# pedrocr/imagepipe

Hardware: AMD Instinct MI355X
Metric: megapixels/sec full raw->sRGB pipe, 100 MP f32 frame (higher is better)
Workload: dtype f32

## Files before the change

bindings/rust/imagepipe_amd_sys.rs:

```rust
#![allow(non_camel_case_types, dead_code)]
use std::os::raw::{c_char, c_int, c_uint, c_void};

pub const IPK_OK: c_int = 0;
pub const IPK_NOOP: c_int = 1;
pub const IPK_ERR_NOT_INIT: c_int = -1;
pub const IPK_ERR_INVALID: c_int = -2;
pub const IPK_ERR_HIP: c_int = -3;
pub const IPK_ERR_NO_DEVICE: c_int = -4;
pub const IPK_ERR_UNSUPPORTED: c_int = -5;
pub const IPK_ERR_NOMEM: c_int = -6;

pub const IPK_OR_NORMAL: c_int = 0;
pub const IPK_OR_HFLIP: c_int = 1;
pub const IPK_OR_ROT180: c_int = 2;
pub const IPK_OR_VFLIP: c_int = 3;
pub const IPK_OR_TRANSPOSE: c_int = 4;
pub const IPK_OR_ROT90: c_int = 5;
pub const IPK_OR_TRANSVERSE: c_int = 6;
pub const IPK_OR_ROT270: c_int = 7;
pub const IPK_OR_UNKNOWN: c_int = 8;

pub const IPK_ROT_NORMAL: c_int = 0;
pub const IPK_ROT_90: c_int = 1;
pub const IPK_ROT_180: c_int = 2;
// ... 230 lines not shown
  pub fn ipk_host_output16bit(src: *const f32, n: usize, dst: *mut u16) -> c_int;
  pub fn ipk_host_raw_to_srgb(p: *const IpkFusedParams, src: *const c_void, dst: *mut c_void) -> c_int;
  pub fn ipk_selftest_cdiv(c: f32, variant: c_int, lo: f32, hi: f32, include_special: c_int, n_bad: *mut u64, first_bad_bits: *mut u32) -> c_int;
  pub fn ipk_selftest_lut_weight(n_bad: *mut u64, first_bad_bits: *mut u32) -> c_int;
  pub fn ipk_selftest_clamp01(n_bad: *mut u64, first_bad_bits: *mut u32) -> c_int;
  pub fn ipk_copy_probe(src: *const c_void, dst: *mut c_void, bytes: usize, stream: *mut c_void) -> c_int;
  pub fn ipk_mix_probe(src: *const c_void, dst: *mut c_void, src_bytes: usize, stream: *mut c_void) -> c_int;
  pub fn ipk_clock_probe(out2_dev: *mut u64, spin_us: u32, stream: *mut c_void) -> c_int;
  pub fn ipk_stream_probe(p: *const IpkFusedParams, src: *const c_void, dst: *mut c_void, stream: *mut c_void) -> c_int;
  pub fn ipk_selftest_spline3(exposure: f32, points: *const f32, npoints: c_int, n_bad: *mut u64, first_bad_bits: *mut u32) -> c_int;
  pub fn ipk_selftest_quant8(variant: c_int, n_bad: *mut u64, first_bad_bits: *mut u32) -> c_int;
  pub fn ipk_selftest_q8(n_bad: *mut u64, first_bad_bits: *mut u32) -> c_int;
  pub fn ipk_selftest_quant16(n_bad: *mut u64, first_bad_bits: *mut u32) -> c_int;
  pub fn ipk_selftest_cbrtf(r#in: *const f32, out: *mut f32, n: usize, variant: c_int, stream: *mut c_void) -> c_int;
  pub fn ipk_selftest_task_queue(enabled: c_int) -> c_int;
  pub fn ipk_selftest_cache_put(cache: *mut IpkCache, key32: *const u8, bytes: usize) -> c_int;
  pub fn ipk_selftest_sha256(data: *const c_void, n: usize, out32: *mut u8) -> c_int;
}
```

imagepipe_amd/_lib.py:

```python
import ctypes as C
import os

_HERE = os.path.dirname(os.path.abspath(__file__))
SO_PATH = os.environ.get("IPK_SO_OVERRIDE") or os.path.join(_HERE, "libimagepipe_amd.so")

IPK_OK, IPK_NOOP = 0, 1
SRC_U16, SRC_F32, SRC_RGB8, SRC_RGB16 = 0, 1, 2, 3
OUT_F32, OUT_U8, OUT_U16 = 0, 1, 2
SCHED_AUTO, SCHED_SPLIT = 0, 1
OR_NORMAL, OR_HFLIP, OR_ROT180, OR_VFLIP, OR_TRANSPOSE, OR_ROT90, OR_TRANSVERSE, OR_ROT270, OR_UNKNOWN = range(9)
ROT_NORMAL, ROT_90, ROT_180, ROT_270 = range(4)

_sz = C.c_size_t
_vp = C.c_void_p
_fp = C.POINTER(C.c_float)
_szp = C.POINTER(C.c_size_t)
_i64 = C.c_int64


class _SizedDesc(C.Structure):

    def __init__(self, *a, **k):
        super().__init__(*a, **k)
        self.struct_size = C.sizeof(self)
# ... 141 lines not shown
    "ipk_host_raw_to_srgb": (C.c_int, [C.POINTER(FusedParams), _vp, _vp]),
    "ipk_selftest_cdiv": (C.c_int, [C.c_float, C.c_int, C.c_float, C.c_float, C.c_int, C.POINTER(C.c_uint64), C.POINTER(C.c_uint32)]),
    "ipk_selftest_lut_weight": (C.c_int, [C.POINTER(C.c_uint64), C.POINTER(C.c_uint32)]),
    "ipk_selftest_clamp01": (C.c_int, [C.POINTER(C.c_uint64), C.POINTER(C.c_uint32)]),
    "ipk_abi_sizeof": (_sz, [C.c_int]),
    "ipk_copy_probe": (C.c_int, [_vp, _vp, _sz, _vp]),
    "ipk_mix_probe": (C.c_int, [_vp, _vp, _sz, _vp]),
    "ipk_clock_probe": (C.c_int, [_vp, C.c_uint32, _vp]),
    "ipk_stream_probe": (C.c_int, [C.POINTER(FusedParams), _vp, _vp, _vp]),
    "ipk_selftest_spline3": (C.c_int, [C.c_float, _fp, C.c_int, C.POINTER(C.c_uint64), C.POINTER(C.c_uint32)]),
    "ipk_selftest_quant8": (C.c_int, [C.c_int, C.POINTER(C.c_uint64), C.POINTER(C.c_uint32)]),
    "ipk_selftest_q8": (C.c_int, [C.POINTER(C.c_uint64), C.POINTER(C.c_uint32)]),
    "ipk_selftest_quant16": (C.c_int, [C.POINTER(C.c_uint64), C.POINTER(C.c_uint32)]),
    "ipk_selftest_cbrtf": (C.c_int, [_vp, _vp, _sz, C.c_int, _vp]),
    "ipk_selftest_task_queue": (C.c_int, [C.c_int]),
    "ipk_selftest_cache_put": (C.c_int, [_vp, C.c_char_p, _sz]),
    "ipk_selftest_sha256": (C.c_int, [C.c_char_p, _sz, C.c_char_p]),
    "ipk_pointwise_chain": (C.c_int, [_vp, _sz, _sz, C.c_int, _fp, _fp, C.c_float, _fp, C.c_int, C.c_int, _vp, _vp]),
    "ipk_pointwise_chain_out": (C.c_int, [_vp, _sz, _sz, C.c_int, _fp, _fp, C.c_float, _fp, C.c_int, C.c_int, C.c_int, _vp, _vp]),
    "ipk_raster_to_srgb": (C.c_int, [_vp, C.c_int, _sz, _sz, _fp, _fp, C.c_float, _fp, C.c_int, C.c_int, C.c_int, _vp, _vp]),
    "ipk_pipeline_takes_fastpath": (C.c_int, [C.POINTER(PipelineDesc), C.c_int]),
    "ipk_pipeline_fuses_rotatecrop": (C.c_int, [C.POINTER(PipelineDesc), C.c_int]),
    "ipk_pipeline_hashes": (C.c_int, [C.POINTER(PipelineDesc), C.c_int, C.c_uint64, C.c_char_p]),
    "ipk_cache_new": (C.c_int, [_sz, C.POINTER(C.c_void_p)]),
    "ipk_cache_free": (C.c_int, [_vp]),
    "ipk_cache_clear": (C.c_int, [_vp]),
    "ipk_cache_contains": (C.c_int, [_vp, C.c_char_p]),
    "ipk_cache_stats": (C.c_int, [_vp, C.POINTER(_sz), C.POINTER(_sz), C.POINTER(C.c_uint64), C.POINTER(C.c_uint64), C.POINTER(C.c_uint64)]),
    "ipk_cache_get": (C.c_int, [_vp, C.c_char_p, C.POINTER(C.c_void_p), C.POINTER(_sz), C.POINTER(_sz), C.POINTER(_sz), C.POINTER(C.c_int)]),
    "ipk_timing_begin": (C.c_int, []),
# ... 52 lines not shown
```

imagepipe_amd/csrc/ipk_api.cpp:

```cpp
#include <hip/hip_runtime_api.h>

#include <algorithm>
#include <cmath>
#include <cstdarg>
#include <cstdio>
#include <cstddef>
#include <cstring>
#include <atomic>
#include <map>
#include <memory>
#include <mutex>
#include <string>
#include <thread>
#include <vector>

#include "../../include/imagepipe_amd.h"
#include "ipk_hash.hpp"
#include "ipk_host.hpp"
#include "ipk_internal.hpp"
#include "ipk_launch.hpp"

namespace {

thread_local char g_err[512] = "";
// ... 1181 lines not shown
  REQUIRE_INIT();
  if (!src || !dst || (bytes & 15) || ((uintptr_t)src & 15) || ((uintptr_t)dst & 15)) return fail(IPK_ERR_INVALID, "ipk_copy_probe wants 16-byte aligned buffers and a multiple of 16 bytes");
  ipk::launch_copy_probe(src, dst, bytes, cx().num_cus, S(stream)); HIPCHK(hipGetLastError());
  return IPK_OK;
}
int ipk_mix_probe(const void *src, void *dst, size_t src_bytes, void *stream) {
  REQUIRE_INIT();
  if (!src || !dst || (src_bytes & 4095) || ((uintptr_t)src & 15) || ((uintptr_t)dst & 15)) return fail(IPK_ERR_INVALID, "ipk_mix_probe wants 16-byte aligned buffers and a multiple of 4096 source bytes (whole blocks)");
  ipk::launch_mix_probe(src, dst, src_bytes, S(stream)); HIPCHK(hipGetLastError());
  return IPK_OK;
}
int ipk_clock_probe(uint64_t *out2_dev, uint32_t spin_us, void *stream) {
  REQUIRE_INIT();
  if (!out2_dev || spin_us == 0 || spin_us > 2000000u) return fail(IPK_ERR_INVALID, "ipk_clock_probe: null output or a spin outside (0, 2 s]");
  ipk::launch_clock_probe(out2_dev, (unsigned long long)spin_us * 100ull, S(stream)); HIPCHK(hipGetLastError());
  return IPK_OK;
}
int ipk_selftest_task_queue(int enabled) { REQUIRE_INIT(); ipk::selftest_task_queue(enabled != 0); return IPK_OK; }
int ipk_selftest_spline3(float exposure, const float *points, int npoints, uint64_t *n_bad, uint32_t *first_bad_bits) {
  REQUIRE_INIT();
  if (!n_bad || (npoints > 0 && !points)) return fail(IPK_ERR_INVALID, "bad selftest arguments");
  ipk::Spline sp; int rc = build_curve(exposure, points, npoints, sp); if (rc) return rc;
  void *dev; rc = selftest_alloc(&dev); if (rc) return rc;
  if (ipk::launch_selftest_spline3(sp, dev, nullptr) != 0) { (void)hipFree(dev); return fail(IPK_ERR_UNSUPPORTED, "the kernels keep the select form for this curve"); }
  HIPCHK(hipGetLastError());
  return selftest_collect(dev, n_bad, first_bad_bits);
}
int ipk_selftest_quant16(uint64_t *n_bad, uint32_t *first_bad_bits) {
  REQUIRE_INIT();
  if (!n_bad) return fail(IPK_ERR_INVALID, "bad selftest arguments");
// ... 1074 lines not shown
```

imagepipe_amd/csrc/ipk_kernels.hip:

```cpp
#include <hip/hip_runtime.h>
#include <stdint.h>
#include <cstring>
#include <cmath>
#include <type_traits>
#include <atomic>
#include <mutex>
#include <utility>
#include <vector>
#include "ipk_device.hpp"
#include "ipk_launch.hpp"

using namespace ipkd;

#define IPK_RARE(x) __builtin_expect(!!(x), 0)
constexpr uint32_t kSpread = 4;
constexpr uint32_t kMinTaskRows = 4;
#ifndef IPK_SPLIT_MIN_ROWS
#define IPK_SPLIT_MIN_ROWS 16u
#endif
constexpr uint32_t kStealMin = 4;

namespace ipk {

typedef LutPair LabTab;
// ... 1203 lines not shown
  uint64_t owidth;
  uint32_t row_off;
  uint32_t out_r0, out_r1;
  uint32_t n_frames;
  uint32_t *task_ctr;
  float min0, range0;
  float inv_range0;
  int exact_norm;
  int fast_ok;
  int xoff, yoff;
  ToLabParams tolab;
  Mat9 rgbm;
  int has_curve, linear;
  uint32_t n_strips, n_segs;
  uint32_t lc_base, lc_rem;
  const float *lab_table;
  const float *gam_table;
  const LutPair *lab_pairs, *gam_pairs;
  const Q8Entry *gam_q8;
  const float *gen_cells;
  uint32_t gen_pw, gen_ph;
  int gen_check;
  int px_guard;
  int ori;
  int roles[4];
  SplineDev spline;
};

struct RowWin { float l, v0, v1, v2, v3, r; };

// ... 572 lines not shown
  __shared__ __attribute__((aligned(16))) uint32_t s_stage[FULL ? 16 * STG : 4];
  if (threadIdx.x < 4) s_par[threadIdx.x] = a.tolab.mul[threadIdx.x];
  else if (threadIdx.x < 16) s_par[threadIdx.x] = a.tolab.cm[threadIdx.x - 4];
  else if (threadIdx.x < 25) s_par[threadIdx.x] = a.rgbm.m[threadIdx.x - 16];
  if (threadIdx.x < kSplineMaxKnots) fill_knots(s_knots, a.spline, (int)threadIdx.x);
  constexpr bool HAS_GRID = CM != 1 && !DEMO && !SKEL;
  __shared__ __attribute__((aligned(16))) float s_grid[HAS_GRID ? kGridFloats : 4];
  if (HAS_GRID && (CM == 2 || a.spline.grid_ok)) fill_grid(s_grid, a.spline, (int)threadIdx.x);
  __shared__ unsigned long long s_tdesc[16];
  __shared__ uint32_t s_tcur[16];
  if ((threadIdx.x & 63u) == 0) { s_tdesc[threadIdx.x >> 6] = 0ull; s_tcur[threadIdx.x >> 6] = 0u; }
  bool arrived = false;
  auto arrive = [&]() { if (!arrived) { sync_after_lds_direct(); arrived = true; } };

  const uint32_t lane = threadIdx.x & 63u;
  const uint32_t per_frame = a.n_strips * a.n_segs;
  const uint32_t n_waves = gridDim.x * (blockDim.x >> 6);
  const uint32_t n_tasks = BATCH ? per_frame * a.n_frames : per_frame;
  auto draw = [&]() -> uint32_t {
    uint32_t t = 0xFFFFFFFFu;
    if ((threadIdx.x & 63u) == 0) {
      t = n_waves + atomicAdd(a.task_ctr, 1u);
    }
    t = (uint32_t)__builtin_amdgcn_readfirstlane((int)t);
    return t;
  };
  const bool queued = a.task_ctr != nullptr && n_tasks > n_waves;
  const uint32_t wslot = threadIdx.x >> 6, nwb = blockDim.x >> 6;
  const bool steal_on = a.n_strips <= 0xFFFFu && (!BATCH || a.n_frames <= 64u);
  uint32_t tserial = 0;
  auto take_over = [&](uint32_t &frame, uint32_t &strip, uint32_t &r0, uint32_t &r1) -> bool {
    for (int attempt = 0; attempt < 4; ++attempt) {
      unsigned long long d = 0ull; uint32_t c = 0u;
// ... 12 lines not shown
      uint32_t ok = 0u;
      if (lane == 0) ok = atomicCAS(&s_tdesc[bl], dv, nv) == dv ? 1u : 0u;
      if (__builtin_amdgcn_readfirstlane((int)ok) != 0) { strip = dhi & 0xFFFFu; frame = (dhi >> 16) & 63u; r0 = mid; r1 = dlo; return true; }
    }
    return false;
  };
  const uint32_t gt0 = queued ? blockIdx.x * (blockDim.x >> 6) + (threadIdx.x >> 6)
                              : (((threadIdx.x >> 6) / kSpread) * gridDim.x + blockIdx.x) * kSpread + ((threadIdx.x >> 6) % kSpread);
  auto next_task = [&](uint32_t gt) -> uint32_t {
    if (gt >= n_tasks) return 0xFFFFFFFFu;
    if (queued) return draw();
    return (n_tasks - gt > n_waves) ? gt + n_waves : 0xFFFFFFFFu;
  };
  for (uint32_t gt = (uint32_t)__builtin_amdgcn_readfirstlane((int)gt0);; gt = next_task(gt)) {
    uint32_t frame = 0u, strip, r0, r1;
    if (gt < n_tasks) {
      frame = BATCH ? (uint32_t)__builtin_amdgcn_readfirstlane((int)(gt / per_frame)) : 0u;
      const uint32_t task = (uint32_t)__builtin_amdgcn_readfirstlane((int)(BATCH ? gt - frame * per_frame : gt));
      strip = task % a.n_strips;
      const uint32_t seg = task / a.n_strips;
      const uint32_t nrows = a.out_r1 - a.out_r0;
      r0 = a.out_r0 + (uint32_t)(((uint64_t)seg * nrows) / a.n_segs);
      r1 = a.out_r0 + (uint32_t)(((uint64_t)(seg + 1) * nrows) / a.n_segs);
    } else {
      arrive();
      if (!steal_on) break;
      if (lane == 0) __hip_atomic_store(&s_tdesc[wslot], (unsigned long long)(++tserial & 0x3FFu) << 54, __ATOMIC_RELAXED, __HIP_MEMORY_SCOPE_WORKGROUP);
      if (__builtin_amdgcn_readfirstlane(take_over(frame, strip, r0, r1) ? 1 : 0) == 0) break;
    }
    strip = (uint32_t)__builtin_amdgcn_readfirstlane((int)strip); r0 = (uint32_t)__builtin_amdgcn_readfirstlane((int)r0); r1 = (uint32_t)__builtin_amdgcn_readfirstlane((int)r1);
    if (BATCH) frame = (uint32_t)__builtin_amdgcn_readfirstlane((int)frame);
    const void *const frame_src = BATCH ? bp->src[frame] : a.src;
    void *const frame_dst = BATCH ? bp->dst[frame] : a.dst;

    const uint32_t lc0 = FULL ? 0u : strip * a.lc_base + min(strip, a.lc_rem);
    const uint32_t nl = FULL ? 64u : a.lc_base + (strip < a.lc_rem ? 1u : 0u);
    const bool lane_on = FULL ? true : lane < nl;
    const uint32_t pc0 = (WIN ? win->x0 : 0u) + (FULL ? min(strip * 256u, (WIN ? win->x1 - win->x0 : a.W) - 256u) : 4u * lc0);
    const bool win_inner = WIN && FULL && pc0 >= win->c0 && pc0 + 256u <= win->c1;
    const uint32_t col0 = pc0 + 4u * min(lane, nl - 1);
    const uint32_t nvalid = FULL ? 4u : min(4u, a.W - col0);
    const uint32_t xo = ((uint32_t)a.xoff + pc0) & 1u;
    uint32_t cxo[4] = {0, 0, 0, 0};
    if (GEN) {
      #pragma unroll
      for (int j = 0; j < 4; ++j) cxo[j] = ((col0 + j) % a.gen_pw) * kGenCellFloats;
    }
    const bool gen_guard = GEN && (sizeof(SrcT) == 4 || DEMO || a.gen_check != 0);
    if (r0 >= r1) { arrive(); continue; }
    if (steal_on && lane == 0) {
      __hip_atomic_store(&s_tdesc[wslot], (unsigned long long)(++tserial & 0x3FFu) << 54, __ATOMIC_RELAXED, __HIP_MEMORY_SCOPE_WORKGROUP);
      __hip_atomic_store(&s_tcur[wslot], r0, __ATOMIC_RELAXED, __HIP_MEMORY_SCOPE_WORKGROUP);
      __hip_atomic_store(&s_tdesc[wslot], ((unsigned long long)(((++tserial & 0x3FFu) << 22) | (frame << 16) | strip) << 32) | r1, __ATOMIC_RELEASE, __HIP_MEMORY_SCOPE_WORKGROUP);
    }

    const bool is_first = lane == 0, is_last = lane + 1 == nl;
    const bool single = FULL ? false : nl == 1;
    const int64_t hcol_want = is_first ? (int64_t)pc0 - 1 : (int64_t)pc0 + 4 * (int64_t)nl;
    const uint32_t hcol = ((is_first || is_last) && hcol_want >= 0 && hcol_want < (int64_t)a.W) ? (uint32_t)hcol_want : col0;
    const uint32_t h2col = (single && pc0 + 4u * nl < a.W) ? pc0 + 4u * nl : col0;

    const SrcT *src = reinterpret_cast<const SrcT *>(frame_src);
    const float min0 = a.min0, range0 = a.range0, inv_range0 = a.inv_range0;
    const bool exact_norm = CMN ? false : a.exact_norm != 0;
    const bool fast_ok = CMN ? true : a.fast_ok != 0, has_curve = CMN ? true : a.has_curve != 0, linear = CMN ? (OUTS == 2) : a.linear != 0;

    struct RawRowT { float v0, v1, v2, v3, h, h2; };
    auto issue_row = [&](uint32_t row) -> RawRowT {
      const SrcT *rp = src + (uint64_t)(row - a.row_off) * a.owidth;
      RawRowT t;
      load_raw4<SrcT, VEC>(rp + col0, nvalid, t.v0, t.v1, t.v2, t.v3);
// ... 41 lines not shown
      } else {
        w.v0 = rs_min(d0 / range0, 1.0f); w.v1 = rs_min(d1 / range0, 1.0f); w.v2 = rs_min(d2 / range0, 1.0f); w.v3 = rs_min(d3 / range0, 1.0f);
        h = rs_min(dh / range0, 1.0f);
        if (single) h2 = rs_min(dh2 / range0, 1.0f);
      }
      if (gen_guard) {
        flag = __builtin_amdgcn_ballot_w64(gen_sample_bad(w.v0) | gen_sample_bad(w.v1) | gen_sample_bad(w.v2) | gen_sample_bad(w.v3) |
                                           gen_sample_bad(h) | gen_sample_bad(h2)) != 0;
        if (flag && !redo) {
          w.v0 = rs_min(d0 / range0, 1.0f); w.v1 = rs_min(d1 / range0, 1.0f); w.v2 = rs_min(d2 / range0, 1.0f); w.v3 = rs_min(d3 / range0, 1.0f);
          h = rs_min(dh / range0, 1.0f);
          if (single) h2 = rs_min(dh2 / range0, 1.0f);
        }
      }
      w.l = dpp_wave_shr1(h, w.v3);
      const float rr = dpp_wave_shl1(h, w.v0);
      w.r = is_last ? (single ? h2 : h) : rr;
      return w;
    };

    const bool store_aligned = (OUTS == 0 || OUTS == 3) ? true : ((OUTS == 1) ? ((a.W & 3u) == 0) : ((a.W & 1u) == 0));
    const uint32_t Hm1 = a.H - 1, Wm1 = a.W - 1;
    const bool col_edge = lane_on && (col0 == 0 || col0 + 3 >= Wm1);

    RowWin P = {0, 0, 0, 0, 0, 0}, C, N = {0, 0, 0, 0, 0, 0};
    bool fP = false, fC = false, fN = false;
    RawRowT raw_next;
    {
      const RawRowT rp = issue_row(r0 > 0 ? r0 - 1 : 0u), rc = issue_row(r0), rn = issue_row(min(r0 + 1, Hm1));
      raw_next = issue_row(min(r0 + 2, Hm1));
      P = finish_row(rp, fP); C = finish_row(rc, fC); N = finish_row(rn, fN);
    }
    arrive();
    uint32_t ry = GEN ? r0 % a.gen_ph : 0u;
    auto compute_px = [&](const RowWin &P, const RowWin &C, const RowWin &N, const bool fP, const bool fC, const bool fN, const uint32_t r, float4 px[4]) {
      const int pr = (int)((r + (uint32_t)a.yoff) & 1u);
      const float pw[6] = {P.l, P.v0, P.v1, P.v2, P.v3, P.r};
      const float cw[6] = {C.l, C.v0, C.v1, C.v2, C.v3, C.r};
      const float nw[6] = {N.l, N.v0, N.v1, N.v2, N.v3, N.r};
      const float *rowcells = s_cells + ry * a.gen_pw * kGenCellFloats;
      if (GEN) {
        const bool literal = fP | fC | fN;
        #pragma unroll
        for (int j = 0; j < 4; ++j) {
          float t[9] = {pw[j], pw[j + 1], pw[j + 2], cw[j], cw[j + 1], cw[j + 2], nw[j], nw[j + 1], nw[j + 2]};
// ... 16 lines not shown
          px[3] = demosaic_inner_px<0, ZA>(pw[3], pw[4], pw[5], cw[3], cw[4], cw[5], nw[3], nw[4], nw[5]);
        }
      } else {
        if (xo == 0) {
          px[0] = demosaic_inner_px<2, ZA>(pw[0], pw[1], pw[2], cw[0], cw[1], cw[2], nw[0], nw[1], nw[2]);
          px[1] = demosaic_inner_px<3, ZA>(pw[1], pw[2], pw[3], cw[1], cw[2], cw[3], nw[1], nw[2], nw[3]);
          px[2] = demosaic_inner_px<2, ZA>(pw[2], pw[3], pw[4], cw[2], cw[3], cw[4], nw[2], nw[3], nw[4]);
          px[3] = demosaic_inner_px<3, ZA>(pw[3], pw[4], pw[5], cw[3], cw[4], cw[5], nw[3], nw[4], nw[5]);
        } else {
          px[0] = demosaic_inner_px<3, ZA>(pw[0], pw[1], pw[2], cw[0], cw[1], cw[2], nw[0], nw[1], nw[2]);
          px[1] = demosaic_inner_px<2, ZA>(pw[1], pw[2], pw[3], cw[1], cw[2], cw[3], nw[1], nw[2], nw[3]);
          px[2] = demosaic_inner_px<3, ZA>(pw[2], pw[3], pw[4], cw[2], cw[3], cw[4], nw[2], nw[3], nw[4]);
          px[3] = demosaic_inner_px<2, ZA>(pw[3], pw[4], pw[5], cw[3], cw[4], cw[5], nw[3], nw[4], nw[5]);
        }
      }
      const bool edge_lane = (r == 0) || (r == Hm1) || col_edge;
      if (IPK_RARE(__builtin_amdgcn_ballot_w64(edge_lane) != 0)) {
        if (edge_lane) {
          #pragma unroll
          for (int j = 0; j < 4; ++j) {
            const uint32_t c = col0 + j;
            if (c < a.W && (r == 0 || r == Hm1 || c == 0 || c == Wm1)) {
              const float t[9] = {pw[j], pw[j + 1], pw[j + 2], cw[j], cw[j + 1], cw[j + 2], nw[j], nw[j + 1], nw[j + 2]};
              uint32_t m = 0x1FFu;
              if (r == 0) m &= ~0x007u;
              if (r == Hm1) m &= ~0x1C0u;
              if (c == 0) m &= ~0x049u;
              if (c == Wm1) m &= ~0x124u;
              if (ROT) {
                float to[9];
                const uint32_t mo = ori_window_dyn(a.ori, pw, cw, nw, j, to, m);
                const int role = a.roles[2 * (int)(r & 1u) + (int)((j + xo) & 1u)];
                px[j] = GEN ? demosaic_gen_literal_px(__float_as_uint(rowcells[cxo[j] + 27]), to, mo) : demosaic_edge_dispatch(to, mo, role >> 1, role & 1);
              } else
              px[j] = GEN ? demosaic_gen_literal_px(__float_as_uint(rowcells[cxo[j] + 27]), t, m) : demosaic_edge_dispatch(t, m, pr, (int)((j + xo) & 1u));
            }
          }
        }
      }
    };
    auto row_step = [&](RowWin &P, RowWin &C, RowWin &N, bool &fP, bool &fC, bool &fN, const uint32_t r) {
// ... 30 lines not shown
        for (int j = 0; j < 4; ++j) { o[j].r = px[j].x; o[j].g = px[j].y; o[j].b = px[j].z; }
      } else {
      bool bad = !fast_ok || (!PXG && sizeof(SrcT) == 4 && (fP | fC | fN));
      if (fast_ok) bad |= pointwise4_fast<PXG>(a, s_par, s_lab, s_gam, s_knots, px, o, has_curve, linear, CM, nullptr, HAS_GRID ? s_grid : nullptr);
      if (IPK_RARE(__builtin_amdgcn_ballot_w64(bad) != 0)) {
        #pragma unroll
        for (int j = 0; j < 4; ++j) {
          const PixOut e = pointwise_exact(a, s_lab, s_gam, s_knots, px[j]);
          if (bad) o[j] = e;
        }
      }
      }
      bool fNN;
      const RowWin NN = finish_row(raw_next, fNN);
      __builtin_amdgcn_sched_barrier(0);
      if (FULL && (!WIN || win_inner)) {
        uint32_t *stg = s_stage + (threadIdx.x >> 6) * STG;
        if constexpr (Q8) OutStage<1>::stage_bits(stg, lane, o); else OutStage<OUTS>::stage(stg, lane, o);
        __builtin_amdgcn_fence(__ATOMIC_RELEASE, "wavefront"); __builtin_amdgcn_wave_barrier(); __builtin_amdgcn_fence(__ATOMIC_ACQUIRE, "wavefront");
        if (WIN) OutStage<OUTS>::flush(stg, lane, frame_dst, (size_t)(r - a.out_r0) * win->pitch + (pc0 - win->c0));
        else OutStage<OUTS>::flush(stg, lane, frame_dst, (size_t)(r - a.out_r0) * a.W + pc0);
        __builtin_amdgcn_fence(__ATOMIC_RELEASE, "wavefront"); __builtin_amdgcn_wave_barrier(); __builtin_amdgcn_fence(__ATOMIC_ACQUIRE, "wavefront");
      } else if (WIN) {
        if (lane_on) win_store<OUTS, Q8>(frame_dst, (size_t)(r - a.out_r0) * win->pitch, col0, win->c0, win->c1, o);
      } else {
        if (lane_on) OutStore<OUTS>::store(frame_dst, (size_t)(r - a.out_r0) * a.W + col0, nvalid, o, store_aligned);
      }
      __builtin_amdgcn_sched_barrier(0);
      raw_next = issue_row(min(r + 3, Hm1));
      P = NN; fP = fNN;
      if (GEN) ry = (ry + 1 == a.gen_ph) ? 0u : ry + 1;
    };
    for (uint32_t r = r0, r1d = r1; r < r1d; ++r) {
      uint32_t e_now = r1;
      if (steal_on) {
        if (lane == 0) __hip_atomic_store(&s_tcur[wslot], r, __ATOMIC_RELAXED, __HIP_MEMORY_SCOPE_WORKGROUP);
        e_now = (uint32_t)__hip_atomic_load(reinterpret_cast<uint32_t *>(&s_tdesc[wslot]), __ATOMIC_RELAXED, __HIP_MEMORY_SCOPE_WORKGROUP);
      }
      row_step(P, C, N, fP, fC, fN, r);
      { const RowWin t = P; P = C; C = N; N = t; const bool ft = fP; fP = fC; fC = fN; fN = ft; }
      if (steal_on) r1d = (uint32_t)__builtin_amdgcn_readfirstlane((int)e_now);
    }
  }
  arrive();
  if (queued && (threadIdx.x & 63u) == 0) {
    uint32_t *const arrived = a.task_ctr + kQueueStride;
    if (atomicAdd(arrived, 1u) == n_waves - 1u) {
      __hip_atomic_store(a.task_ctr, 0u, __ATOMIC_RELAXED, __HIP_MEMORY_SCOPE_AGENT);
      __hip_atomic_store(arrived, 0u, __ATOMIC_RELAXED, __HIP_MEMORY_SCOPE_AGENT);
    }
  }
}
template <typename SrcT, bool VEC, int OUT, bool FULL, bool GEN, bool PXG = true, int CM = 0, bool ROT = false>
__global__ __launch_bounds__(1024) void k_fused_bayer(FusedArgs a) { fused_bayer_body<SrcT, VEC, OUT, FULL, GEN, PXG, CM, ROT, false>(a, nullptr); }
template <typename SrcT, bool VEC, int OUT, bool PXG>
__global__ __launch_bounds__(1024) void k_fused_bayer_batch(FusedArgs a, BatchPtrs bp) { fused_bayer_body<SrcT, VEC, OUT, true, false, PXG, 1, false, true>(a, &bp); }
template <typename SrcT, bool VEC, int OUT, bool FULL, bool GEN, bool PXG, int CM>
__global__ __launch_bounds__(1024) void k_fused_bayer_window(FusedArgs a, FusedWindow w) { fused_bayer_body<SrcT, VEC, OUT, FULL, GEN, PXG, CM, false, false, true>(a, nullptr, &w); }

static void fused_task_grid(FusedArgs &a, int num_cus, unsigned &blocks, uint32_t frames = 1, uint32_t waves_per_block = 16);
static bool task_counters_for(TaskQueues *q, hipStream_t s, FusedArgs &a, std::unique_lock<std::mutex> &lk);
static int launch_status() { return hipGetLastError() == hipSuccess ? 0 : -4; }

int launch_demosaic_bayer(const float *src, size_t width, size_t img_height, size_t src_row0, size_t out_row0, size_t out_rows,
                          int xoff, int yoff, const float *gen_cells, int gen_pw, int gen_ph, float *dst4, int num_cus, TaskQueues *queues, hipStream_t s) {
  FusedArgs a;
  std::memset(&a, 0, sizeof(a));
  a.src = src; a.dst = dst4; a.W = (uint32_t)width; a.H = (uint32_t)img_height; a.owidth = width;
  a.row_off = (uint32_t)src_row0; a.out_r0 = (uint32_t)out_row0; a.out_r1 = (uint32_t)(out_row0 + out_rows);
  a.xoff = xoff; a.yoff = yoff; a.range0 = 1.0f; a.inv_range0 = 1.0f;
  a.gen_cells = gen_cells; a.gen_pw = (uint32_t)gen_pw; a.gen_ph = (uint32_t)gen_ph;
  unsigned blocks;
  std::unique_lock<std::mutex> queue_lock;
  (void)task_counters_for(queues, s, a, queue_lock);
  fused_task_grid(a, gen_cells ? num_cus : 2 * (num_cus > 0 ? num_cus : 256), blocks);
// ... 118 lines not shown
        older_than = cand->last_use;
        const hipError_t qs = hipStreamQuery(cand->stream);
        (void)hipGetLastError();
        if (qs != hipErrorNotReady) lru = cand;
      }
      if (!lru) return false;
      lru->key = key; lru->stream = s;
      e = lru;
    }
  }
  e->last_use = ++q->clock;
  a.task_ctr = q->block + (size_t)e->slot * kCtrSlotWords;
  return true;
}

static void fused_task_grid(FusedArgs &a, int num_cus, unsigned &blocks, uint32_t frames, uint32_t waves_per_block) {
  const uint32_t uni = 32u, share_min = frames == 1 ? 128u : 64u;
  const uint32_t grid = (uint32_t)(num_cus > 0 ? num_cus : 256);
  const uint32_t total_waves = grid * waves_per_block;
  const uint32_t w4 = (a.W + 3) / 4;
  a.n_strips = (w4 + 63) / 64;
  a.lc_base = w4 / a.n_strips; a.lc_rem = w4 % a.n_strips;
  const uint32_t nrows = a.out_r1 - a.out_r0;
  const uint64_t share = (uint64_t)nrows * a.n_strips * frames / total_waves;
  if (share >= share_min && a.task_ctr != nullptr) a.n_segs = std::max(1u, nrows / uni);
  else {
    const uint32_t min_rows = kMinTaskRows;
    a.n_segs = std::min(nrows, std::min(std::max(1u, (uint32_t)(total_waves / ((uint64_t)a.n_strips * frames))), std::max(1u, nrows / min_rows)));
  }
  const uint64_t tasks = (uint64_t)a.n_strips * a.n_segs * frames;
  const bool drawn = share >= share_min && a.task_ctr != nullptr;
  const uint64_t per_block = !drawn ? (uint64_t)kSpread : waves_per_block;
  blocks = (unsigned)std::min<uint64_t>(grid, (tasks + per_block - 1) / per_block);
}

int launch_fused_bayer(const FusedLaunch &f, hipStream_t s) {
  FusedArgs a;
  a.src = f.src; a.dst = f.dst; a.W = (uint32_t)f.width; a.H = (uint32_t)f.height; a.owidth = f.owidth;
  a.row_off = (uint32_t)f.row_off; a.out_r0 = (uint32_t)f.out_r0; a.out_r1 = (uint32_t)f.out_r1;
  a.min0 = f.black0; a.range0 = f.white0 - f.black0;
  a.inv_range0 = 1.0f / a.range0;
  a.exact_norm = f.exact_norm;
  a.fast_ok = f.fast_ok;
  a.xoff = f.xoff; a.yoff = f.yoff;
  a.tolab = make_tolab(f.mul4, f.cm12);
  for (int i = 0; i < 9; ++i) a.rgbm.m[i] = f.rgbm9[i];
  a.has_curve = f.has_curve; a.linear = f.linear;
  if (f.has_curve) a.spline = make_spline(*f.spline); else { a.spline.npoints = 0; a.spline.nseg = 0; a.spline.grid_ok = 0; }
// ... 56 lines not shown
        if (!f.src_is_u16) { if (f.out_type == 0) IPK_BATCH_LAUNCH(float, true, 0); else if (f.out_type == 1) IPK_BATCH_LAUNCH(float, true, 1); else IPK_BATCH_LAUNCH(float, true, 2); }
        else { if (f.out_type == 0) IPK_BATCH_LAUNCH(uint16_t, false, 0); else if (f.out_type == 1) IPK_BATCH_LAUNCH(uint16_t, false, 1); else IPK_BATCH_LAUNCH(uint16_t, false, 2); }
#undef IPK_BATCH_LAUNCH
        if (const int rc = launch_status()) return rc;
      } else {
        FusedLaunch one = f;
        one.batch_n = 0;
        for (int i = 0; i < n; ++i) { one.src = f.batch_src[i0 + i]; one.dst = f.batch_dst[i0 + i]; const int rc = launch_fused_bayer(one, s); if (rc) return rc; }
      }
    }
    return 0;
  }
  std::unique_lock<std::mutex> queue_lock;
  (void)task_counters_for(f.queues, s, a, queue_lock);
  unsigned blocks;
  fused_task_grid(a, f.num_cus, blocks);
  if (f.schedule == 1 && a.n_strips * a.n_segs <= (uint32_t)(f.num_cus > 0 ? f.num_cus : 256) * 16u && (a.out_r1 - a.out_r0) / a.n_segs >= IPK_SPLIT_MIN_ROWS) {
    a.n_segs *= 2u; a.task_ctr = nullptr;
  }
  if (f.out_type == 4) {
    if (a.gen_cells || a.ori != 0 || a.W < 256u || a.exact_norm || std::fabs(a.min0) < 0x1p-70f || std::fabs(a.min0) > 0x1p70f) return -2;
    if (!f.src_is_u16) hipLaunchKernelGGL((k_fused_bayer<float, true, 4, true, false, false, true>), dim3(blocks), dim3(1024), 0, s, a);
    else hipLaunchKernelGGL((k_fused_bayer<uint16_t, false, 4, true, false, false, true>), dim3(blocks), dim3(1024), 0, s, a);
    return launch_status();
  }
  if (!f.src_is_u16) {
    if (f.out_type == 0) launch_fused_t<float, true, 0>(a, blocks, s);
    else if (f.out_type == 1) launch_fused_t<float, true, 1>(a, blocks, s);
    else launch_fused_t<float, true, 2>(a, blocks, s);
  } else if (vec) {
    if (f.out_type == 0) launch_fused_t<uint16_t, true, 0>(a, blocks, s);
    else if (f.out_type == 1) launch_fused_t<uint16_t, true, 1>(a, blocks, s);
    else launch_fused_t<uint16_t, true, 2>(a, blocks, s);
// ... 640 lines not shown
```

imagepipe_amd/csrc/ipk_launch.hpp:

```cpp
#pragma once
#include <hip/hip_runtime_api.h>
#include <cstddef>
#include <cstdint>
#include "ipk_host.hpp"

namespace ipk {

typedef Spline SplineHost;

struct TaskQueues;
TaskQueues *create_task_queues();
void destroy_task_queues(TaskQueues *q);

template <typename T>
void launch_gofloat_cfa(const T *src, size_t owidth, size_t x, size_t y, size_t w, size_t h, float black0, float white0,
                        float *dst, hipStream_t s);
template <typename T>
void launch_gofloat_mono(const T *src, size_t owidth, size_t x, size_t y, size_t w, size_t h, float black0, float white0,
                         float *dst4, hipStream_t s);
template <typename T>
void launch_gofloat_rgb(const T *src, size_t owidth, size_t x, size_t y, size_t w, size_t h, const float *black4, const float *white4,
                        float *dst4, hipStream_t s);
void launch_gofloat_other_u8(const uint8_t *src, size_t owidth, size_t x, size_t y, size_t w, size_t h,
                             const void *gamma_reverse_pairs, float *dst4, hipStream_t s);
// ... 46 lines not shown
  int out_type;
  const void *lab_table, *gam_table;
  const void *lab_pairs, *gam_pairs;
  const void *gam_q8;
  int px_guard;
  const float *gen_cells; int gen_pw, gen_ph, gen_check;
  int num_cus;
  int schedule;
  TaskQueues *queues;
  int ori;
  int roles[4];
  int batch_n; const void *const *batch_src; void *const *batch_dst;
  size_t win_c0 = 0, win_c1 = 0;
};
int launch_fused_bayer(const FusedLaunch &f, hipStream_t s);
int launch_fused_resample(const FusedLaunch &f, const ResamplePlan &plan, size_t nwidth, size_t nheight, const uint32_t *lookups_dev, hipStream_t s);
template <typename T>
void launch_rotate1(const T *src, size_t owidth, size_t oheight, int64_t base_offset, int64_t x_step, int64_t y_step, T *dst, hipStream_t s);
int launch_pointwise_chain(const FusedLaunch &f, size_t npix, hipStream_t s);
int launch_tolab_fast(const FusedLaunch &f, size_t npix, hipStream_t s);
int launch_chain_quantised(const FusedLaunch &f, size_t npix, hipStream_t s);
int launch_raster_chain(const FusedLaunch &f, size_t npix, int src_is_u16, const void *gamma_reverse_pairs, hipStream_t s);

int launch_selftest_cdiv(float c, int variant, unsigned lo_bits, unsigned hi_bits, int include_special, void *out_dev, hipStream_t s);
void launch_copy_probe(const void *src, void *dst, size_t bytes, int num_cus, hipStream_t s);
void launch_mix_probe(const void *src, void *dst, size_t src_bytes, hipStream_t s);
void launch_clock_probe(void *out2_dev, unsigned long long spin_ticks, hipStream_t s);
int launch_selftest_spline3(const SplineHost &h, void *out_dev, hipStream_t s);
int launch_selftest_fract(void *out_dev, hipStream_t s);
int launch_selftest_clamp(void *out_dev, hipStream_t s);
// ... 8 lines not shown
```

include/imagepipe_amd.h:

```cpp
#ifndef IMAGEPIPE_AMD_H
#define IMAGEPIPE_AMD_H

#include <stddef.h>
#include <stdint.h>

#ifdef __cplusplus
extern "C" {
#endif

#define IPK_API __attribute__((visibility("default")))

typedef enum {
  IPK_OK = 0,
  IPK_NOOP = 1,
  IPK_ERR_NOT_INIT = -1,
  IPK_ERR_INVALID = -2,
  IPK_ERR_HIP = -3,
  IPK_ERR_NO_DEVICE = -4,
  IPK_ERR_UNSUPPORTED = -5,
  IPK_ERR_NOMEM = -6
} ipk_status;

typedef enum {
  IPK_OR_NORMAL = 0, IPK_OR_HFLIP = 1, IPK_OR_ROT180 = 2, IPK_OR_VFLIP = 3, IPK_OR_TRANSPOSE = 4,
// ... 274 lines not shown

IPK_API int ipk_selftest_cdiv(float c, int variant, float lo, float hi, int include_special,
                              uint64_t *n_bad, uint32_t *first_bad_bits);
IPK_API int ipk_selftest_lut_weight(uint64_t *n_bad, uint32_t *first_bad_bits);
IPK_API int ipk_selftest_clamp01(uint64_t *n_bad, uint32_t *first_bad_bits);
IPK_API int ipk_copy_probe(const void *src, void *dst, size_t bytes, void *stream);
IPK_API int ipk_mix_probe(const void *src, void *dst, size_t src_bytes, void *stream);
IPK_API int ipk_clock_probe(uint64_t *out2_dev, uint32_t spin_us, void *stream);
IPK_API int ipk_stream_probe(const ipk_fused_params *p, const void *src, void *dst, void *stream);
IPK_API int ipk_selftest_spline3(float exposure, const float *points, int npoints, uint64_t *n_bad, uint32_t *first_bad_bits);
IPK_API int ipk_selftest_quant8(int variant, uint64_t *n_bad, uint32_t *first_bad_bits);
IPK_API int ipk_selftest_q8(uint64_t *n_bad, uint32_t *first_bad_bits);
IPK_API int ipk_selftest_quant16(uint64_t *n_bad, uint32_t *first_bad_bits);
IPK_API int ipk_selftest_cbrtf(const float *in, float *out, size_t n, int variant, void *stream);
IPK_API int ipk_selftest_task_queue(int enabled);
IPK_API int ipk_selftest_cache_put(ipk_cache *cache, const uint8_t *key32, size_t bytes);
IPK_API int ipk_selftest_sha256(const void *data, size_t n, uint8_t *out32);

#ifdef __cplusplus
}
#endif
#endif
```

Measured before the change: 215,000.

## Fold narrow right-edge column remainder into packed multi-segment wave tasks

Result: slower. 200,000 (-7.0%).

```diff
diff --git a/bindings/rust/imagepipe_amd_sys.rs b/bindings/rust/imagepipe_amd_sys.rs
--- a/bindings/rust/imagepipe_amd_sys.rs
+++ b/bindings/rust/imagepipe_amd_sys.rs
@@ -268,6 +268,7 @@
   pub fn ipk_selftest_quant16(n_bad: *mut u64, first_bad_bits: *mut u32) -> c_int;
   pub fn ipk_selftest_cbrtf(r#in: *const f32, out: *mut f32, n: usize, variant: c_int, stream: *mut c_void) -> c_int;
   pub fn ipk_selftest_task_queue(enabled: c_int) -> c_int;
+  pub fn ipk_fused_task_plan(width: usize, row0: usize, row1: usize, num_cus: c_int, queued: c_int, schedule: c_int, info: *mut u32, tasks: *mut u32, max_tasks: usize) -> c_int;
   pub fn ipk_selftest_cache_put(cache: *mut IpkCache, key32: *const u8, bytes: usize) -> c_int;
   pub fn ipk_selftest_sha256(data: *const c_void, n: usize, out32: *mut u8) -> c_int;
 }
diff --git a/imagepipe_amd/_lib.py b/imagepipe_amd/_lib.py
--- a/imagepipe_amd/_lib.py
+++ b/imagepipe_amd/_lib.py
@@ -179,6 +179,7 @@
     "ipk_selftest_quant16": (C.c_int, [C.POINTER(C.c_uint64), C.POINTER(C.c_uint32)]),
     "ipk_selftest_cbrtf": (C.c_int, [_vp, _vp, _sz, C.c_int, _vp]),
     "ipk_selftest_task_queue": (C.c_int, [C.c_int]),
+    "ipk_fused_task_plan": (C.c_int, [C.c_size_t, C.c_size_t, C.c_size_t, C.c_int, C.c_int, C.c_int, C.POINTER(C.c_uint32), C.POINTER(C.c_uint32), C.c_size_t]),
     "ipk_selftest_cache_put": (C.c_int, [_vp, C.c_char_p, _sz]),
     "ipk_selftest_sha256": (C.c_int, [C.c_char_p, _sz, C.c_char_p]),
     "ipk_pointwise_chain": (C.c_int, [_vp, _sz, _sz, C.c_int, _fp, _fp, C.c_float, _fp, C.c_int, C.c_int, _vp, _vp]),
diff --git a/imagepipe_amd/csrc/ipk_api.cpp b/imagepipe_amd/csrc/ipk_api.cpp
--- a/imagepipe_amd/csrc/ipk_api.cpp
+++ b/imagepipe_amd/csrc/ipk_api.cpp
@@ -1219,6 +1219,11 @@
   REQUIRE_INIT();
   if (!out2_dev || spin_us == 0 || spin_us > 2000000u) return fail(IPK_ERR_INVALID, "ipk_clock_probe: null output or a spin outside (0, 2 s]");
   ipk::launch_clock_probe(out2_dev, (unsigned long long)spin_us * 100ull, S(stream)); HIPCHK(hipGetLastError());
+  return IPK_OK;
+}
+int ipk_fused_task_plan(size_t width, size_t row0, size_t row1, int num_cus, int queued, int schedule, uint32_t *info, uint32_t *tasks, size_t max_tasks) {
+  if (!info || (schedule != IPK_SCHED_AUTO && schedule != IPK_SCHED_SPLIT)) return fail(IPK_ERR_INVALID, "bad argument");
+  if (ipk::fused_task_plan(width, row0, row1, num_cus, queued != 0, schedule, info, tasks, max_tasks) != 0) return fail(IPK_ERR_INVALID, "bad geometry");
   return IPK_OK;
 }
 int ipk_selftest_task_queue(int enabled) { REQUIRE_INIT(); ipk::selftest_task_queue(enabled != 0); return IPK_OK; }
diff --git a/imagepipe_amd/csrc/ipk_kernels.hip b/imagepipe_amd/csrc/ipk_kernels.hip
--- a/imagepipe_amd/csrc/ipk_kernels.hip
+++ b/imagepipe_amd/csrc/ipk_kernels.hip
@@ -1241,6 +1241,7 @@
   int has_curve, linear;
   uint32_t n_strips, n_segs;
   uint32_t lc_base, lc_rem;
+  uint32_t fold_q, fold_rsh, fold_n, n_fold;
   const float *lab_table;
   const float *gam_table;
   const LutPair *lab_pairs, *gam_pairs;
@@ -1843,9 +1844,10 @@
   auto arrive = [&]() { if (!arrived) { sync_after_lds_direct(); arrived = true; } };
 
   const uint32_t lane = threadIdx.x & 63u;
+  constexpr bool FOLDABLE = FULL && !GEN && !WIN && !BATCH && !DEMO;
   const uint32_t per_frame = a.n_strips * a.n_segs;
   const uint32_t n_waves = gridDim.x * (blockDim.x >> 6);
-  const uint32_t n_tasks = BATCH ? per_frame * a.n_frames : per_frame;
+  const uint32_t n_tasks = BATCH ? per_frame * a.n_frames : per_frame + (FOLDABLE ? a.n_fold : 0u);
   auto draw = [&]() -> uint32_t {
     uint32_t t = 0xFFFFFFFFu;
     if ((threadIdx.x & 63u) == 0) {
@@ -1888,14 +1890,21 @@
   };
   for (uint32_t gt = (uint32_t)__builtin_amdgcn_readfirstlane((int)gt0);; gt = next_task(gt)) {
     uint32_t frame = 0u, strip, r0, r1;
+    bool fold = false;
     if (gt < n_tasks) {
       frame = BATCH ? (uint32_t)__builtin_amdgcn_readfirstlane((int)(gt / per_frame)) : 0u;
       const uint32_t task = (uint32_t)__builtin_amdgcn_readfirstlane((int)(BATCH ? gt - frame * per_frame : gt));
+      if (FOLDABLE && task >= per_frame) {
+        fold = true; strip = a.n_strips;
+        r0 = a.out_r0 + (task - per_frame) * (a.fold_n << a.fold_rsh);
+        r1 = min(r0 + a.fold_n, a.out_r1);
+      } else {
       strip = task % a.n_strips;
       const uint32_t seg = task / a.n_strips;
       const uint32_t nrows = a.out_r1 - a.out_r0;
       r0 = a.out_r0 + (uint32_t)(((uint64_t)seg * nrows) / a.n_segs);
       r1 = a.out_r0 + (uint32_t)(((uint64_t)(seg + 1) * nrows) / a.n_segs);
+      }
     } else {
       arrive();
       if (!steal_on) break;
@@ -1904,15 +1913,26 @@
     }
     strip = (uint32_t)__builtin_amdgcn_readfirstlane((int)strip); r0 = (uint32_t)__builtin_amdgcn_readfirstlane((int)r0); r1 = (uint32_t)__builtin_amdgcn_readfirstlane((int)r1);
     if (BATCH) frame = (uint32_t)__builtin_amdgcn_readfirstlane((int)frame);
+    auto run_task = [&](auto fold_c) __attribute__((always_inline)) {
+    constexpr bool FOLD = decltype(fold_c)::value;
+    uint32_t fli = lane, lofs = 0u;
+    bool fact = true;
+    if constexpr (FOLD) {
+      uint32_t fg = lane / a.fold_q;
+      fli = lane - fg * a.fold_q;
+      fact = fg < (1u << a.fold_rsh);
+      if (!fact) { fg = (1u << a.fold_rsh) - 1u; fli = a.fold_q - 1u; }
+      lofs = fg * a.fold_n;
+    }
     const void *const frame_src = BATCH ? bp->src[frame] : a.src;
     void *const frame_dst = BATCH ? bp->dst[frame] : a.dst;
 
     const uint32_t lc0 = FULL ? 0u : strip * a.lc_base + min(strip, a.lc_rem);
-    const uint32_t nl = FULL ? 64u : a.lc_base + (strip < a.lc_rem ? 1u : 0u);
+    const uint32_t nl = FOLD ? a.fold_q : FULL ? 64u : a.lc_base + (strip < a.lc_rem ? 1u : 0u);
     const bool lane_on = FULL ? true : lane < nl;
-    const uint32_t pc0 = (WIN ? win->x0 : 0u) + (FULL ? min(strip * 256u, (WIN ? win->x1 - win->x0 : a.W) - 256u) : 4u * lc0);
+    const uint32_t pc0 = FOLD ? a.W - 4u * a.fold_q : (WIN ? win->x0 : 0u) + (FULL ? min(strip * 256u, (WIN ? win->x1 - win->x0 : a.W) - 256u) : 4u * lc0);
     const bool win_inner = WIN && FULL && pc0 >= win->c0 && pc0 + 256u <= win->c1;
-    const uint32_t col0 = pc0 + 4u * min(lane, nl - 1);
+    const uint32_t col0 = pc0 + 4u * (FOLD ? fli : min(lane, nl - 1));
     const uint32_t nvalid = FULL ? 4u : min(4u, a.W - col0);
     const uint32_t xo = ((uint32_t)a.xoff + pc0) & 1u;
     uint32_t cxo[4] = {0, 0, 0, 0};
@@ -1921,14 +1941,15 @@
       for (int j = 0; j < 4; ++j) cxo[j] = ((col0 + j) % a.gen_pw) * kGenCellFloats;
     }
     const bool gen_guard = GEN && (sizeof(SrcT) == 4 || DEMO || a.gen_check != 0);
-    if (r0 >= r1) { arrive(); continue; }
-    if (steal_on && lane == 0) {
+    if (r0 >= r1) { arrive(); return; }
+    if (FOLD && steal_on && lane == 0) __hip_atomic_store(&s_tdesc[wslot], (unsigned long long)(++tserial & 0x3FFu) << 54, __ATOMIC_RELAXED, __HIP_MEMORY_SCOPE_WORKGROUP);
+    if (!FOLD && steal_on && lane == 0) {
       __hip_atomic_store(&s_tdesc[wslot], (unsigned long long)(++tserial & 0x3FFu) << 54, __ATOMIC_RELAXED, __HIP_MEMORY_SCOPE_WORKGROUP);
       __hip_atomic_store(&s_tcur[wslot], r0, __ATOMIC_RELAXED, __HIP_MEMORY_SCOPE_WORKGROUP);
       __hip_atomic_store(&s_tdesc[wslot], ((unsigned long long)(((++tserial & 0x3FFu) << 22) | (frame << 16) | strip) << 32) | r1, __ATOMIC_RELEASE, __HIP_MEMORY_SCOPE_WORKGROUP);
     }
 
-    const bool is_first = lane == 0, is_last = lane + 1 == nl;
+    const bool is_first = (FOLD ? fli : lane) == 0, is_last = (FOLD ? fli : lane) + 1 == nl;
     const bool single = FULL ? false : nl == 1;
     const int64_t hcol_want = is_first ? (int64_t)pc0 - 1 : (int64_t)pc0 + 4 * (int64_t)nl;
     const uint32_t hcol = ((is_first || is_last) && hcol_want >= 0 && hcol_want < (int64_t)a.W) ? (uint32_t)hcol_want : col0;
@@ -2000,6 +2021,7 @@
         }
       }
       w.l = dpp_wave_shr1(h, w.v3);
+      if (FOLD) w.l = is_first ? h : w.l;
       const float rr = dpp_wave_shl1(h, w.v0);
       w.r = is_last ? (single ? h2 : h) : rr;
       return w;
@@ -2007,14 +2029,16 @@
 
     const bool store_aligned = (OUTS == 0 || OUTS == 3) ? true : ((OUTS == 1) ? ((a.W & 3u) == 0) : ((a.W & 1u) == 0));
     const uint32_t Hm1 = a.H - 1, Wm1 = a.W - 1;
+    const uint32_t rmax = min(Hm1, a.out_r1);
+    auto frow = [&](uint32_t r, int k) -> uint32_t { return (uint32_t)min(max((int)(r + lofs) + k, 0), (int)rmax); };
     const bool col_edge = lane_on && (col0 == 0 || col0 + 3 >= Wm1);
 
     RowWin P = {0, 0, 0, 0, 0, 0}, C, N = {0, 0, 0, 0, 0, 0};
     bool fP = false, fC = false, fN = false;
     RawRowT raw_next;
     {
-      const RawRowT rp = issue_row(r0 > 0 ? r0 - 1 : 0u), rc = issue_row(r0), rn = issue_row(min(r0 + 1, Hm1));
-      raw_next = issue_row(min(r0 + 2, Hm1));
+      const RawRowT rp = issue_row(FOLD ? frow(r0, -1) : (r0 > 0 ? r0 - 1 : 0u)), rc = issue_row(FOLD ? frow(r0, 0) : r0), rn = issue_row(FOLD ? frow(r0, 1) : min(r0 + 1, Hm1));
+      raw_next = issue_row(FOLD ? frow(r0, 2) : min(r0 + 2, Hm1));
       P = finish_row(rp, fP); C = finish_row(rc, fC); N = finish_row(rn, fN);
     }
     arrive();
@@ -2061,17 +2085,18 @@
           px[3] = demosaic_inner_px<2, ZA>(pw[3], pw[4], pw[5], cw[3], cw[4], cw[5], nw[3], nw[4], nw[5]);
         }
       }
-      const bool edge_lane = (r == 0) || (r == Hm1) || col_edge;
+      const uint32_t re = FOLD ? r + lofs : r;
+      const bool edge_lane = (re == 0) || (re == Hm1) || col_edge;
       if (IPK_RARE(__builtin_amdgcn_ballot_w64(edge_lane) != 0)) {
         if (edge_lane) {
           #pragma unroll
           for (int j = 0; j < 4; ++j) {
             const uint32_t c = col0 + j;
-            if (c < a.W && (r == 0 || r == Hm1 || c == 0 || c == Wm1)) {
+            if (c < a.W && (re == 0 || re == Hm1 || c == 0 || c == Wm1)) {
               const float t[9] = {pw[j], pw[j + 1], pw[j + 2], cw[j], cw[j + 1], cw[j + 2], nw[j], nw[j + 1], nw[j + 2]};
               uint32_t m = 0x1FFu;
-              if (r == 0) m &= ~0x007u;
-              if (r == Hm1) m &= ~0x1C0u;
+              if (re == 0) m &= ~0x007u;
+              if (re == Hm1) m &= ~0x1C0u;
               if (c == 0) m &= ~0x049u;
               if (c == Wm1) m &= ~0x124u;
               if (ROT) {
@@ -2132,7 +2157,9 @@
       bool fNN;
       const RowWin NN = finish_row(raw_next, fNN);
       __builtin_amdgcn_sched_barrier(0);
-      if (FULL && (!WIN || win_inner)) {
+      if constexpr (FOLD) {
+        if (fact && r + lofs < a.out_r1) win_store<OUTS, Q8>(frame_dst, (size_t)(r + lofs - a.out_r0) * a.W, col0, 0u, a.W, o);
+      } else if (FULL && (!WIN || win_inner)) {
         uint32_t *stg = s_stage + (threadIdx.x >> 6) * STG;
         if constexpr (Q8) OutStage<1>::stage_bits(stg, lane, o); else OutStage<OUTS>::stage(stg, lane, o);
         __builtin_amdgcn_fence(__ATOMIC_RELEASE, "wavefront"); __builtin_amdgcn_wave_barrier(); __builtin_amdgcn_fence(__ATOMIC_ACQUIRE, "wavefront");
@@ -2145,20 +2172,23 @@
         if (lane_on) OutStore<OUTS>::store(frame_dst, (size_t)(r - a.out_r0) * a.W + col0, nvalid, o, store_aligned);
       }
       __builtin_amdgcn_sched_barrier(0);
-      raw_next = issue_row(min(r + 3, Hm1));
+      raw_next = issue_row(FOLD ? frow(r, 3) : min(r + 3, Hm1));
       P = NN; fP = fNN;
       if (GEN) ry = (ry + 1 == a.gen_ph) ? 0u : ry + 1;
     };
     for (uint32_t r = r0, r1d = r1; r < r1d; ++r) {
       uint32_t e_now = r1;
-      if (steal_on) {
+      if (steal_on && !FOLD) {
         if (lane == 0) __hip_atomic_store(&s_tcur[wslot], r, __ATOMIC_RELAXED, __HIP_MEMORY_SCOPE_WORKGROUP);
         e_now = (uint32_t)__hip_atomic_load(reinterpret_cast<uint32_t *>(&s_tdesc[wslot]), __ATOMIC_RELAXED, __HIP_MEMORY_SCOPE_WORKGROUP);
       }
       row_step(P, C, N, fP, fC, fN, r);
       { const RowWin t = P; P = C; C = N; N = t; const bool ft = fP; fP = fC; fC = fN; fN = ft; }
-      if (steal_on) r1d = (uint32_t)__builtin_amdgcn_readfirstlane((int)e_now);
-    }
+      if (steal_on && !FOLD) r1d = (uint32_t)__builtin_amdgcn_readfirstlane((int)e_now);
+    }
+    };
+    if constexpr (FOLDABLE) { if (fold) run_task(std::true_type{}); else run_task(std::false_type{}); }
+    else run_task(std::false_type{});
   }
   arrive();
   if (queued && (threadIdx.x & 63u) == 0) {
@@ -2176,7 +2206,7 @@
 template <typename SrcT, bool VEC, int OUT, bool FULL, bool GEN, bool PXG, int CM>
 __global__ __launch_bounds__(1024) void k_fused_bayer_window(FusedArgs a, FusedWindow w) { fused_bayer_body<SrcT, VEC, OUT, FULL, GEN, PXG, CM, false, false, true>(a, nullptr, &w); }
 
-static void fused_task_grid(FusedArgs &a, int num_cus, unsigned &blocks, uint32_t frames = 1, uint32_t waves_per_block = 16);
+static void fused_task_grid(FusedArgs &a, int num_cus, unsigned &blocks, uint32_t frames = 1, uint32_t waves_per_block = 16, bool fold_ok = false);
 static bool task_counters_for(TaskQueues *q, hipStream_t s, FusedArgs &a, std::unique_lock<std::mutex> &lk);
 static int launch_status() { return hipGetLastError() == hipSuccess ? 0 : -4; }
 
@@ -2325,12 +2355,24 @@
   return true;
 }
 
-static void fused_task_grid(FusedArgs &a, int num_cus, unsigned &blocks, uint32_t frames, uint32_t waves_per_block) {
+static void fused_fold_plan(FusedArgs &a) {
+  const uint32_t nrows = a.out_r1 - a.out_r0, longest = (nrows + a.n_segs - 1) / a.n_segs;
+  a.fold_rsh = 0;
+  while ((2u << a.fold_rsh) * a.fold_q <= 64u) ++a.fold_rsh;
+  a.fold_n = std::max(2u, longest & ~1u);
+  const uint64_t per_task = (uint64_t)a.fold_n << a.fold_rsh;
+  a.n_fold = (uint32_t)((nrows + per_task - 1) / per_task);
+}
+static void fused_task_grid(FusedArgs &a, int num_cus, unsigned &blocks, uint32_t frames, uint32_t waves_per_block, bool fold_ok) {
   const uint32_t uni = 32u, share_min = frames == 1 ? 128u : 64u;
   const uint32_t grid = (uint32_t)(num_cus > 0 ? num_cus : 256);
   const uint32_t total_waves = grid * waves_per_block;
   const uint32_t w4 = (a.W + 3) / 4;
   a.n_strips = (w4 + 63) / 64;
+  a.fold_q = a.fold_rsh = a.fold_n = a.n_fold = 0;
+  const uint32_t full = a.W / 256u, left = (a.W - 256u * full + 3u) / 4u;
+  const bool folded = fold_ok && frames == 1 && full >= 1u && left >= 1u && left <= 32u;
+  if (folded) { a.n_strips = full; a.fold_q = left; }
   a.lc_base = w4 / a.n_strips; a.lc_rem = w4 % a.n_strips;
   const uint32_t nrows = a.out_r1 - a.out_r0;
   const uint64_t share = (uint64_t)nrows * a.n_strips * frames / total_waves;
@@ -2338,11 +2380,47 @@
   else {
     const uint32_t min_rows = kMinTaskRows;
     a.n_segs = std::min(nrows, std::min(std::max(1u, (uint32_t)(total_waves / ((uint64_t)a.n_strips * frames))), std::max(1u, nrows / min_rows)));
-  }
-  const uint64_t tasks = (uint64_t)a.n_strips * a.n_segs * frames;
+    if (folded) for (fused_fold_plan(a); (uint64_t)a.n_strips * a.n_segs + a.n_fold > total_waves && a.n_segs > 1u; fused_fold_plan(a)) --a.n_segs;
+  }
+  if (folded) fused_fold_plan(a);
+  const uint64_t tasks = (uint64_t)a.n_strips * a.n_segs * frames + a.n_fold;
   const bool drawn = share >= share_min && a.task_ctr != nullptr;
   const uint64_t per_block = !drawn ? (uint64_t)kSpread : waves_per_block;
   blocks = (unsigned)std::min<uint64_t>(grid, (tasks + per_block - 1) / per_block);
+}
+
+int fused_task_plan(size_t width, size_t out_r0, size_t out_r1, int num_cus, bool queued, int schedule, uint32_t info[8], uint32_t *tasks, size_t max_tasks) {
+  if (width < 1 || width > 0xFFFFFFFFull || out_r1 > 0xFFFFFFFFull || out_r0 >= out_r1) return -1;
+  FusedArgs a;
+  std::memset(&a, 0, sizeof(a));
+  a.W = (uint32_t)width; a.out_r0 = (uint32_t)out_r0; a.out_r1 = (uint32_t)out_r1;
+  uint32_t dummy = 0;
+  a.task_ctr = queued ? &dummy : nullptr;
+  unsigned blocks;
+  fused_task_grid(a, num_cus, blocks, 1, 16, a.W >= 256u);
+  if (schedule == 1 && a.n_strips * a.n_segs <= (uint32_t)(num_cus > 0 ? num_cus : 256) * 16u && (a.out_r1 - a.out_r0) / a.n_segs >= IPK_SPLIT_MIN_ROWS) {
+    a.n_segs *= 2u; a.task_ctr = nullptr;
+    if (a.n_fold) fused_fold_plan(a);
+  }
+  const uint32_t per_frame = a.n_strips * a.n_segs, n_tasks = per_frame + a.n_fold, nrows = a.out_r1 - a.out_r0;
+  info[0] = a.n_strips; info[1] = a.n_segs; info[2] = a.n_fold; info[3] = a.fold_q; info[4] = 1u << a.fold_rsh; info[5] = a.fold_n;
+  info[6] = blocks; info[7] = n_tasks;
+  const bool full = a.W >= 256u;
+  for (uint32_t t = 0; tasks && t < n_tasks && t < max_tasks; ++t) {
+    uint32_t *o = tasks + 6 * (size_t)t;
+    if (t >= per_frame) {
+      const uint32_t r0 = a.out_r0 + (t - per_frame) * (a.fold_n << a.fold_rsh), r1 = std::min(r0 + a.fold_n, a.out_r1);
+      const uint64_t end = std::min<uint64_t>((uint64_t)r0 + ((uint64_t)a.fold_n << a.fold_rsh), a.out_r1);
+      o[0] = a.W - 4u * a.fold_q; o[1] = a.W; o[2] = r0; o[3] = (uint32_t)end; o[4] = r1 - r0; o[5] = 1;
+    } else {
+      const uint32_t strip = t % a.n_strips, seg = t / a.n_strips;
+      const uint32_t r0 = a.out_r0 + (uint32_t)(((uint64_t)seg * nrows) / a.n_segs), r1 = a.out_r0 + (uint32_t)(((uint64_t)(seg + 1) * nrows) / a.n_segs);
+      const uint32_t lc0 = strip * a.lc_base + std::min(strip, a.lc_rem), nl = a.lc_base + (strip < a.lc_rem ? 1u : 0u);
+      const uint32_t pc0 = full ? std::min(strip * 256u, a.W - 256u) : 4u * lc0;
+      o[0] = pc0; o[1] = full ? pc0 + 256u : std::min(a.W, pc0 + 4u * nl); o[2] = r0; o[3] = r1; o[4] = r1 - r0; o[5] = 0;
+    }
+  }
+  return 0;
 }
 
 int launch_fused_bayer(const FusedLaunch &f, hipStream_t s) {
@@ -2429,9 +2507,10 @@
   std::unique_lock<std::mutex> queue_lock;
   (void)task_counters_for(f.queues, s, a, queue_lock);
   unsigned blocks;
-  fused_task_grid(a, f.num_cus, blocks);
+  fused_task_grid(a, f.num_cus, blocks, 1, 16, !a.gen_cells && a.W >= 256u);
   if (f.schedule == 1 && a.n_strips * a.n_segs <= (uint32_t)(f.num_cus > 0 ? f.num_cus : 256) * 16u && (a.out_r1 - a.out_r0) / a.n_segs >= IPK_SPLIT_MIN_ROWS) {
     a.n_segs *= 2u; a.task_ctr = nullptr;
+    if (a.n_fold) fused_fold_plan(a);
   }
   if (f.out_type == 4) {
     if (a.gen_cells || a.ori != 0 || a.W < 256u || a.exact_norm || std::fabs(a.min0) < 0x1p-70f || std::fabs(a.min0) > 0x1p70f) return -2;
diff --git a/imagepipe_amd/csrc/ipk_launch.hpp b/imagepipe_amd/csrc/ipk_launch.hpp
--- a/imagepipe_amd/csrc/ipk_launch.hpp
+++ b/imagepipe_amd/csrc/ipk_launch.hpp
@@ -84,6 +84,7 @@
   size_t win_c0 = 0, win_c1 = 0;
 };
 int launch_fused_bayer(const FusedLaunch &f, hipStream_t s);
+int fused_task_plan(size_t width, size_t out_r0, size_t out_r1, int num_cus, bool queued, int schedule, uint32_t info[8], uint32_t *tasks, size_t max_tasks);
 int launch_fused_resample(const FusedLaunch &f, const ResamplePlan &plan, size_t nwidth, size_t nheight, const uint32_t *lookups_dev, hipStream_t s);
 template <typename T>
 void launch_rotate1(const T *src, size_t owidth, size_t oheight, int64_t base_offset, int64_t x_step, int64_t y_step, T *dst, hipStream_t s);
diff --git a/include/imagepipe_amd.h b/include/imagepipe_amd.h
--- a/include/imagepipe_amd.h
+++ b/include/imagepipe_amd.h
@@ -312,6 +312,7 @@
 IPK_API int ipk_selftest_quant16(uint64_t *n_bad, uint32_t *first_bad_bits);
 IPK_API int ipk_selftest_cbrtf(const float *in, float *out, size_t n, int variant, void *stream);
 IPK_API int ipk_selftest_task_queue(int enabled);
+IPK_API int ipk_fused_task_plan(size_t width, size_t row0, size_t row1, int num_cus, int queued, int schedule, uint32_t *info, uint32_t *tasks, size_t max_tasks);
 IPK_API int ipk_selftest_cache_put(ipk_cache *cache, const uint8_t *key32, size_t bytes);
 IPK_API int ipk_selftest_sha256(const void *data, size_t n, uint8_t *out32);
 
```
